# vlongle/pixie

Measured on NVIDIA H100. Metric: unet_voxels_per_s, higher is better.
Workload: dtype fp16e5 (U-Net, fp32 accumulate) + f32 (MPM)

## Files before the change

pixie_b200/csrc/conv3d_igemm.cu:

```cuda
#include "conv3d_igemm.cuh"
#include "ptx.cuh"

#include <algorithm>
#include <cmath>
#include <cstdio>
#include <cstring>

#include <cuda_fp8.h>

namespace pixie {

using namespace ptx;

namespace {

constexpr int kMaxWStages = 4;
constexpr int kMaxSStages = 8;
constexpr int kConsumerWarps = 8;
constexpr int kProducerWarp = 8;

struct SmemCtrl {
    uint64_t wfull[kMaxWStages];
    uint64_t wempty[kMaxWStages];
    uint64_t sfull[kMaxSStages];
    uint64_t sempty[kMaxSStages];
    int abort_flag;
};

constexpr int kCtlBarrierBytes = 512;
constexpr int kCmChunk = 16;
constexpr int kCmStageLd = 68;
constexpr int kCmStageFloats = kCmChunk * kCmStageLd;
constexpr int kStatsMaxC = 256;

struct TileCoord {
    int nb, d0, h0, w0, n0, ph_begin, ph_end, split, tde;
};

__device__ __forceinline__ TileCoord decode_tile(const ConvKernelParams& p, int wi) {
    TileCoord t;
    unsigned rest = (unsigned)wi;
    if (p.split_k == 1) {
        t.split = 0; t.ph_begin = 0; t.ph_end = p.n_phases;
    } else {
        const unsigned sk = (unsigned)p.split_k;
        t.split = (int)(rest % sk);
        rest /= sk;
        t.ph_begin = (int)(((unsigned)t.split * (unsigned)p.n_phases) / sk);
        t.ph_end = (int)((((unsigned)t.split + 1u) * (unsigned)p.n_phases) / sk);
    }
    const unsigned nt = rest % (unsigned)p.n_tiles;
    unsigned m = rest / (unsigned)p.n_tiles;
    const unsigned tw = m % (unsigned)p.tiles_w;
    m /= (unsigned)p.tiles_w;
    const unsigned th = m % (unsigned)p.tiles_h;
    m /= (unsigned)p.tiles_h;
    const unsigned td = m % (unsigned)p.tiles_d;
    t.nb = (int)(m / (unsigned)p.tiles_d);
    t.d0 = (int)td * p.TD;
    t.h0 = (int)th * p.TH;
    t.w0 = (int)tw * p.TW;
    t.n0 = (int)nt * p.block_n;
    t.tde = min(p.TD, p.D - t.d0);
    return t;
}

template <int N, bool F8>
__device__ __forceinline__ void mma_block(float* acc, uint32_t a, uint32_t b) {
    wgmma_fence();
#pragma unroll
    for (int k4 = 0; k4 < 4; ++k4) {
        const uint64_t da = make_sw128_desc(a + 32u * k4), db = make_sw128_desc(b + 32u * k4);
        if (F8) {
            if (N == 16) wgmma_e5m2_n16(acc, da, db);
            if (N == 32) wgmma_e5m2_n32(acc, da, db);
            if (N == 64) wgmma_e5m2_n64(acc, da, db);
            if (N == 128) wgmma_e5m2_n128(acc, da, db);
            if (N == 256) wgmma_e5m2_n256(acc, da, db);
        } else {
            if (N == 16) wgmma_f16_n16(acc, da, db);
            if (N == 32) wgmma_f16_n32(acc, da, db);
            if (N == 64) wgmma_f16_n64(acc, da, db);
            if (N == 128) wgmma_f16_n128(acc, da, db);
            if (N == 256) wgmma_f16_n256(acc, da, db);
        }
    }
    wgmma_commit();
}

__device__ __forceinline__ void wgmma_wait_n(int n) {
    switch (n) {
        case 0: wgmma_wait<0>(); break;
        case 1: wgmma_wait<1>(); break;
        case 2: wgmma_wait<2>(); break;
        case 3: wgmma_wait<3>(); break;
        case 4: wgmma_wait<4>(); break;
        case 5: wgmma_wait<5>(); break;
        case 6: wgmma_wait<6>(); break;
        case 7: wgmma_wait<7>(); break;
        case 8: wgmma_wait<8>(); break;
        case 9: wgmma_wait<9>(); break;
        default: wgmma_wait<0>(); break;
    }
}

struct RingPos {
    int stage = 0, parity = 0;
    __device__ __forceinline__ void advance(int n_stages) {
        if (++stage == n_stages) { stage = 0; parity ^= 1; }
    }
};

struct PendingStages {
    int s = -1, w = -1;
    __device__ __forceinline__ void release(SmemCtrl* ctl, int lane) {
        if (lane == 0) {
            if (s >= 0) mbar_arrive(&ctl->sempty[s]);
            if (w >= 0) mbar_arrive(&ctl->wempty[w]);
        }
        s = -1; w = -1;
    }
};

struct ConvStats {
    float* rows;
    int nb = -1;
    double tot_s = 0.0, tot_q = 0.0;

    __device__ __forceinline__ void flush(const ConvKernelParams& p, int lane) {
        if (p.stats_scalar) {
#pragma unroll
            for (int off = 16; off >= 1; off >>= 1) {
                tot_s += __shfl_xor_sync(0xffffffffu, tot_s, off);
                tot_q += __shfl_xor_sync(0xffffffffu, tot_q, off);
            }
            if (lane == 0) {
                atomicAdd(p.stats + (size_t)nb * p.Cout * 2, tot_s);
                atomicAdd(p.stats + (size_t)nb * p.Cout * 2 + 1, tot_q);
            }
            tot_s = 0.0; tot_q = 0.0;
            return;
        }
        asm volatile("bar.sync 1, 256;" ::: "memory");
        for (int ch = threadIdx.x; ch < p.Cout; ch += 256) {
            atomicAdd(p.stats + ((size_t)nb * p.Cout + ch) * 2, (double)rows[ch]);
            atomicAdd(p.stats + ((size_t)nb * p.Cout + ch) * 2 + 1, (double)rows[p.stats_ld + ch]);
            rows[ch] = 0.f;
            rows[p.stats_ld + ch] = 0.f;
        }
        asm volatile("bar.sync 1, 256;" ::: "memory");
    }
    __device__ __forceinline__ void enter(const ConvKernelParams& p, int item_nb, int lane) {
        if (nb != item_nb) {
            if (nb >= 0) flush(p, lane);
            nb = item_nb;
        }
    }
};

struct ConvSmem {
    uint8_t* w;
    uint8_t* s;
    SmemCtrl* ctl;
    float* stage;
    float* stats;
};

__device__ __forceinline__ ConvSmem conv_prologue(const ConvKernelParams& p, int stage_floats, int n_threads) {
    extern __shared__ __align__(1024) uint8_t smem_raw[];
    uint8_t* smem = reinterpret_cast<uint8_t*>(
        (reinterpret_cast<uintptr_t>(smem_raw) + 1023) & ~static_cast<uintptr_t>(1023));
    ConvSmem m;
    m.w = smem;
    m.s = smem + (size_t)p.w_stages * p.w_stage_bytes;
    m.ctl = reinterpret_cast<SmemCtrl*>(m.s + (size_t)p.s_stages * p.s_stage_bytes);
// ... 109 lines not shown
        RingPos wring, sring;
        const uint32_t w_base0 = smem_u32(sm.w), s_base0 = smem_u32(sm.s) + (uint32_t)(g * 64 * 128);
        bool ok = true;
        const long long DHW = (long long)p.D * p.H * p.W;
        ConvStats stats{sm.stats};
        int th2[2], tw2[2];
#pragma unroll
        for (int r2 = 0; r2 < 2; ++r2) {
            const int r = g * 64 + wq * 16 + (lane >> 2) + 8 * r2;
            th2[r2] = r / p.TW; tw2[r2] = r % p.TW;
        }
        const int cq = (lane & 3) * 2;

        for (int wi = blockIdx.x; wi < total_items && ok; wi += gridDim.x) {
            const TileCoord t = decode_tile(p, wi);
#pragma unroll
            for (int d = 0; d < TD; ++d)
#pragma unroll
                for (int j = 0; j < BN / 2; ++j) acc[d][j] = 0.f;
            PendingStages pend;
            int prev_f8 = -1;
            for (int ph = t.ph_begin; ph < t.ph_end && ok; ++ph) {
                const ConvPhase P = p.phases[ph];
                const int n_kd = P.n_kd, n_kh = P.n_kh;
                const bool f8 = P.f8 != 0;
                if (prev_f8 >= 0 && prev_f8 != (int)f8) wgmma_wait<0>();
                prev_f8 = (int)f8;
                ok = mbar_wait(&ctl->wfull[wring.stage], wring.parity, abort_flag);
                if (!ok) break;
                const uint32_t w_addr = w_base0 + (uint32_t)(wring.stage * p.w_stage_bytes);
                const int nplanes = t.tde + n_kd - 1;
                for (int pl = 0; pl < nplanes && ok; ++pl) {
                    ok = mbar_wait(&ctl->sfull[sring.stage], sring.parity, abort_flag);
                    if (!ok) break;
                    const int d_min = max(0, pl - (n_kd - 1)), d_max = min(t.tde - 1, pl);
                    const int groups = issue_slab<BN, TD>(acc, s_base0 + (uint32_t)(sring.stage * p.s_stage_bytes), w_addr, pl, d_min,
                                                          d_max, n_kd, n_kh, p.TW, f8);
                    wgmma_wait_n(groups);
                    pend.release(ctl, lane);
                    pend.s = sring.stage;
                    sring.advance(p.s_stages);
                }
                pend.w = wring.stage;
                wring.advance(p.w_stages);
                if (p.w_stages == 1) { wgmma_wait<0>(); pend.release(ctl, lane); }
            }
            wgmma_wait<0>();
            pend.release(ctl, lane);
#pragma unroll
            for (int d = 0; d < TD; ++d)
#pragma unroll
                for (int j = 0; j < BN / 2; ++j) fence_operand(acc[d][j]);
            if (!ok) break;

            if (do_stats) stats.enter(p, t.nb, lane);
            const bool first_split = (t.split == 0);
            const bool use_bias = first_split && p.bias != nullptr;
            const bool use_res = first_split && p.residual != nullptr;
#pragma unroll
            for (int d = 0; d < TD; ++d) {
                if (d >= t.tde) break;
#pragma unroll
                for (int r2 = 0; r2 < 2; ++r2) {
                    const int hh = t.h0 + th2[r2], ww = t.w0 + tw2[r2];
                    const bool row_ok = (hh < p.H) && (ww < p.W);
                    const long long vox = ((long long)(t.d0 + d) * p.H + hh) * p.W + ww;
#pragma unroll
                    for (int j8 = 0; j8 < BN / 8; ++j8) {
                        const int ch = t.n0 + j8 * 8 + cq;
                        float& a0 = acc[d][j8 * 4 + r2 * 2];
                        float& a1 = acc[d][j8 * 4 + r2 * 2 + 1];
                        const bool ok0 = row_ok && ch < p.Cout, ok1 = row_ok && ch + 1 < p.Cout;
                        float v0 = a0, v1 = a1;
                        if (use_bias) {
                            if (ok0) v0 += __ldg(p.bias + ch);
                            if (ok1) v1 += __ldg(p.bias + ch + 1);
                        }
                        if (p.out_planar) {
                            const long long i0 = ((long long)t.nb * p.Cout + ch) * DHW + vox;
                            if (ok0) {
                                if (use_res) v0 += p.residual[i0];
                                if (p.atomic_out) atomicAdd(p.out + i0, v0); else p.out[i0] = v0;
                            }
                            if (ok1) {
                                if (use_res) v1 += p.residual[i0 + DHW];
                                if (p.atomic_out) atomicAdd(p.out + i0 + DHW, v1); else p.out[i0 + DHW] = v1;
                            }
                        } else if (ok0) {
                            const long long base = ((long long)t.nb * DHW + vox) * p.out_ld + p.out_c0 + ch;
                            if (ok1 && (base & 1) == 0) {
                                if (use_res) {
                                    const float2 rv = __ldg(reinterpret_cast<const float2*>(p.residual + base));
                                    v0 += rv.x; v1 += rv.y;
                                }
                                if (p.atomic_out) red_add_v2(p.out + base, v0, v1);
                                else *reinterpret_cast<float2*>(p.out + base) = make_float2(v0, v1);
                            } else {
                                if (use_res) { v0 += p.residual[base]; if (ok1) v1 += p.residual[base + 1]; }
                                if (p.atomic_out) { atomicAdd(p.out + base, v0); if (ok1) atomicAdd(p.out + base + 1, v1); }
                                else { p.out[base] = v0; if (ok1) p.out[base + 1] = v1; }
                            }
                        }
                        a0 = ok0 ? v0 : 0.f;
                        a1 = ok1 ? v1 : 0.f;
                    }
                }
            }
            if (do_stats) {
                if (scalar_stats) {
                    float s = 0.f, q2 = 0.f;
#pragma unroll
                    for (int d = 0; d < TD; ++d)
#pragma unroll
                        for (int j = 0; j < BN / 2; ++j) { s += acc[d][j]; q2 = fmaf(acc[d][j], acc[d][j], q2); }
                    stats.tot_s += (double)s; stats.tot_q += (double)q2;
                } else {
#pragma unroll
                    for (int j8 = 0; j8 < BN / 8; ++j8)
#pragma unroll
                        for (int e = 0; e < 2; ++e) {
                            float s = 0.f, q2 = 0.f;
#pragma unroll
                            for (int d = 0; d < TD; ++d)
#pragma unroll
                                for (int r2 = 0; r2 < 2; ++r2) {
                                    const float v = acc[d][j8 * 4 + r2 * 2 + e];
                                    s += v; q2 = fmaf(v, v, q2);
                                }
#pragma unroll
                            for (int off = 4; off <= 16; off <<= 1) {
                                s += __shfl_xor_sync(0xffffffffu, s, off);
                                q2 += __shfl_xor_sync(0xffffffffu, q2, off);
                            }
                            const int ch = t.n0 + j8 * 8 + cq + e;
                            if (lane < 4 && ch < p.Cout) {
                                atomicAdd(stats.rows + ch, s);
                                atomicAdd(stats.rows + p.stats_ld + ch, q2);
                            }
                        }
                }
            }
        }
        if (do_stats && stats.nb >= 0 && ok) stats.flush(p, lane);
    }

    conv_report_abort(p, ctl);
}

template <int NV>
__global__ void __launch_bounds__(kConvCmThreads, 1)
conv3d_igemm_cm_kernel(const __grid_constant__ ConvKernelParams p) {
    constexpr int TW = NV == 64 ? 8 : 16;
    const ConvSmem sm = conv_prologue(p, 2 * kCmStageFloats, kConvCmThreads);
// ... 23 lines not shown
            const TileCoord t = decode_tile(p, wi);
#pragma unroll
            for (int j = 0; j < NV / 2; ++j) acc[j] = 0.f;
            const bool has_plane = g < t.tde;
            PendingStages pend;
            int prev_f8 = -1;
            for (int ph = t.ph_begin; ph < t.ph_end && ok; ++ph) {
                const ConvPhase P = p.phases[ph];
                const int n_kd = P.n_kd, n_kh = P.n_kh;
                const bool f8 = P.f8 != 0;
                if (prev_f8 >= 0 && prev_f8 != (int)f8) wgmma_wait<0>();
                prev_f8 = (int)f8;
                const int w0 = wring.stage;
                const int nplanes = t.tde + n_kd - 1;
                for (int pl = 0; pl < nplanes && ok; ++pl) {
                    if (pl < n_kd) {
                        ok = mbar_wait(&ctl->wfull[wring.stage], wring.parity, abort_flag);
                        if (!ok) break;
                        wring.advance(p.w_stages);
                    }
                    ok = mbar_wait(&ctl->sfull[sring.stage], sring.parity, abort_flag);
                    if (!ok) break;
                    const int kd = pl - g;
                    int groups = 0;
                    if (has_plane && kd >= 0 && kd < n_kd) {
                        int wsk = w0 + kd;
                        if (wsk >= p.w_stages) wsk -= p.w_stages;
                        const uint32_t w_addr = w_base0 + (uint32_t)(wsk * p.w_stage_bytes);
                        const uint32_t s_addr = s_base0 + (uint32_t)(sring.stage * p.s_stage_bytes);
                        for (int kh = 0; kh < n_kh; ++kh) {
                            const uint32_t a = w_addr + (uint32_t)(conv_wtile(0, 1, kh, 0) * 64 * 128);
                            const uint32_t b = s_addr + (uint32_t)(kh * TW * 128);
                            if (f8) mma_block<NV, true>(acc, a, b);
                            else mma_block<NV, false>(acc, a, b);
                            ++groups;
                        }
                    }
                    wgmma_wait_n(groups);
                    pend.release(ctl, lane);
                    pend.s = sring.stage;
                    const int kd_done = pl - t.tde + 1;
                    if (kd_done >= 0) {
                        pend.w = w0 + kd_done;
                        if (pend.w >= p.w_stages) pend.w -= p.w_stages;
                    }
                    sring.advance(p.s_stages);
                }
            }
            wgmma_wait<0>();
            pend.release(ctl, lane);
#pragma unroll
            for (int j = 0; j < NV / 2; ++j) fence_operand(acc[j]);
            if (!ok) break;

            if (do_stats) stats.enter(p, t.nb, lane);
            if (!has_plane) continue;
            const bool first_split = (t.split == 0);
            const int ch = t.n0 + 4 * q4;
            const bool ch_ok = ch < p.Cout;
            float4 bias4 = make_float4(0.f, 0.f, 0.f, 0.f);
            if (first_split && p.bias != nullptr && ch_ok)
                bias4 = make_float4(__ldg(p.bias + ch), __ldg(p.bias + ch + 1), __ldg(p.bias + ch + 2), __ldg(p.bias + ch + 3));
            const bool use_res = first_split && p.residual != nullptr;
            const long long plane_base = ((long long)t.nb * p.D + t.d0 + g) * p.H;
            float st_s[4] = {0.f, 0.f, 0.f, 0.f}, st_q[4] = {0.f, 0.f, 0.f, 0.f};
#pragma unroll
            for (int c = 0; c < NV / kCmChunk; ++c) {
#pragma unroll
                for (int jj = 0; jj < kCmChunk / 8; ++jj)
#pragma unroll
                    for (int r2 = 0; r2 < 2; ++r2)
#pragma unroll
                        for (int e = 0; e < 2; ++e) {
                            const int row = wq * 16 + (lane >> 2) + 8 * r2, v = jj * 8 + (lane & 3) * 2 + e;
                            stage[v * kCmStageLd + row] = acc[(c * (kCmChunk / 8) + jj) * 4 + r2 * 2 + e];
                        }
                asm volatile("bar.sync %0, 128;" ::"r"(2 + g) : "memory");
#pragma unroll
                for (int k = 0; k < kCmChunk / 8; ++k) {
                    const int v = vr + 8 * k, vt = c * kCmChunk + v;
                    const int hh = t.h0 + vt / TW, ww = t.w0 + vt % TW;
                    float4 x = *reinterpret_cast<const float4*>(stage + v * kCmStageLd + 4 * q4);
                    if (ch_ok && hh < p.H && ww < p.W) {
                        const long long base = ((plane_base + hh) * p.W + ww) * p.out_ld + p.out_c0 + ch;
                        x.x += bias4.x; x.y += bias4.y; x.z += bias4.z; x.w += bias4.w;
                        if (use_res) {
                            const float4 rv = __ldg(reinterpret_cast<const float4*>(p.residual + base));
                            x.x += rv.x; x.y += rv.y; x.z += rv.z; x.w += rv.w;
                        }
                        if (p.atomic_out) red_add_v4(p.out + base, x.x, x.y, x.z, x.w);
                        else *reinterpret_cast<float4*>(p.out + base) = x;
                        st_s[0] += x.x; st_s[1] += x.y; st_s[2] += x.z; st_s[3] += x.w;
                        st_q[0] = fmaf(x.x, x.x, st_q[0]); st_q[1] = fmaf(x.y, x.y, st_q[1]);
                        st_q[2] = fmaf(x.z, x.z, st_q[2]); st_q[3] = fmaf(x.w, x.w, st_q[3]);
                    }
                }
                asm volatile("bar.sync %0, 128;" ::"r"(2 + g) : "memory");
            }
            if (do_stats) {
                if (scalar_stats) {
                    stats.tot_s += (double)(st_s[0] + st_s[1] + st_s[2] + st_s[3]);
                    stats.tot_q += (double)(st_q[0] + st_q[1] + st_q[2] + st_q[3]);
                } else {
#pragma unroll
                    for (int i = 0; i < 4; ++i) {
                        st_s[i] += __shfl_xor_sync(0xffffffffu, st_s[i], 16);
                        st_q[i] += __shfl_xor_sync(0xffffffffu, st_q[i], 16);
                    }
                    if (lane < 16 && ch_ok) {
#pragma unroll
                        for (int i = 0; i < 4; ++i) {
                            atomicAdd(stats.rows + ch + i, st_s[i]);
                            atomicAdd(stats.rows + p.stats_ld + ch + i, st_q[i]);
                        }
                    }
                }
            }
        }
        if (do_stats && stats.nb >= 0 && ok) stats.flush(p, lane);
    }

    conv_report_abort(p, ctl);
}


int conv_k_total(const ConvDesc& d) {
    int k = 0;
    for (const auto& s : d.segs) k += s.ks * s.ks * s.ks * d.srcs[s.src].C;
    return k;
}

struct SrcSlot { int src; int n_kh; };

static std::vector<SrcSlot> conv_src_slots(const ConvDesc& d) {
    std::vector<SrcSlot> slots;
    for (const auto& s : d.segs) {
        const int n_kh = (s.ks == 3 && d.stride == 1) ? 3 : 1;
        bool found = false;
        for (const auto& sl : slots) found |= (sl.src == s.src && sl.n_kh == n_kh);
        if (!found) slots.push_back({s.src, n_kh});
    }
    return slots;
}

// ... 205 lines not shown

static bool vm_stages(const ConvKernelParams& p, int avail, int& ws, int& ss) {
    ws = (2 * p.w_stage_bytes + 2 * p.s_stage_bytes <= avail) ? 2 : 1;
    if (ws * p.w_stage_bytes + 2 * p.s_stage_bytes > avail) return false;
    ss = std::min(std::min(kMaxSStages, 6), (avail - ws * p.w_stage_bytes) / p.s_stage_bytes);
    return true;
}

int conv_plan_create(const ConvDesc& d, int* d_err_flag, ConvPlan& plan, char* err, int errlen) {
    auto fail = [&](const char* m) { snprintf(err, errlen, "conv_plan_create: %s", m); return 1; };
    PFN_encodeTiled enc = get_encode_fn();
    if (!enc) return fail("cuTensorMapEncodeTiled unavailable (no CUDA driver?)");
    if (d.srcs.empty() || d.segs.empty()) return fail("no sources/segments");
    for (const auto& s : d.srcs)
        if (s.C % 64) return fail("source channels must be a multiple of 64");
    if (d.Cout_pad % 16 || d.Cout_pad < d.Cout) return fail("Cout_pad must be a multiple of 16 >= Cout");

    ConvKernelParams& p = plan.p;
    memset(&p, 0, sizeof(p));
    p.NB = d.NB; p.D = d.D; p.H = d.H; p.W = d.W; p.stride = d.stride;
    p.Cout = d.Cout;
    const int out_ld = d.out_ld ? d.out_ld : d.Cout;

    const auto slots = conv_src_slots(d);
    if ((int)slots.size() > kConvMaxSrc) return fail("too many (source, tap-class) slots");
    const std::vector<ConvPhase> phases = conv_build_phases(d);
    p.n_phases = (int)phases.size();
    int max_taps = 1, max_kh = 1, max_kd = 1;
    bool any3 = false;
    for (const auto& P : phases) {
        max_taps = std::max(max_taps, P.n_kh * P.n_kd);
        max_kh = std::max(max_kh, (int)P.n_kh);
        max_kd = std::max(max_kd, (int)P.n_kd);
        any3 |= (P.n_kh == 3);
    }

    int dev = 0, sms = 132;
    cudaGetDevice(&dev);
    cudaDeviceGetAttribute(&sms, cudaDevAttrMultiProcessorCount, dev);

    plan.channel_major = d.Cout >= 64 && d.Cout % 4 == 0 && !d.out_planar && out_ld % 4 == 0 && d.out_c0 % 4 == 0 &&
                         reinterpret_cast<uintptr_t>(d.out) % 16 == 0 && reinterpret_cast<uintptr_t>(d.residual) % 16 == 0;
    const char* bad = plan.channel_major ? cm_geometry(d, sms, max_kh, p) : vm_geometry(d, sms, any3, max_taps, p);
    if (bad) return fail(bad);
    p.n_tiles = (d.Cout_pad + p.block_n - 1) / p.block_n;
    p.tiles_w = (d.W + p.TW - 1) / p.TW;
    p.tiles_h = (d.H + p.TH - 1) / p.TH;
    p.tiles_d = (d.D + p.TD - 1) / p.TD;

    const int items = conv_work_items(d.NB, p.tiles_d, p.tiles_h, p.tiles_w, p.n_tiles, 1);
    int split = d.split_k;
    if (split <= 0) {
        split = 1;
        while (items * split < 120 && split * 2 <= p.n_phases && split < 64) split *= 2;
    }
    split = std::max(1, std::min(split, p.n_phases));
    if ((long long)p.n_phases * (split + 1) >= (1ll << 31)) return fail("too many phases for the split-K bookkeeping");
    p.split_k = split;
    p.atomic_out = split > 1;
    plan.needs_zero = split > 1;

    for (size_t i = 0; i < slots.size(); ++i) p.slab_rows[i] = p.TW * (p.TH + slots[i].n_kh - 1);
    int max_rows = 0;
    for (size_t i = 0; i < slots.size(); ++i) max_rows = std::max(max_rows, p.slab_rows[i]);
    p.s_stage_bytes = max_rows * 128;
    plan.fused_stats = d.stats != nullptr && split == 1 && d.Cout <= kStatsMaxC && !d.out_planar;
    p.stats_ld = (d.Cout + 31) / 32 * 32;
    const int stats_bytes = plan.fused_stats ? 2 * p.stats_ld * 4 : 0;
    const int ctl_core = kCtlBarrierBytes + (plan.channel_major ? 2 * kCmStageFloats * 4 : 0) + stats_bytes;
    auto plan_stages = [&](int slack, int& ws, int& ss) {
        const int avail = 227 * 1024 - ctl_core - slack;
        return plan.channel_major ? cm_stages(p, max_kd, avail, ws, ss) : vm_stages(p, avail, ws, ss);
    };
    int ws1 = 0, ss1 = 0, ws0 = 0, ss0 = 0;
    const bool ok1 = plan_stages(1024, ws1, ss1), ok0 = plan_stages(0, ws0, ss0);
    if (!ok0) return fail("tile does not fit in shared memory");
    if (ok1 && ws1 >= ws0 && ss1 >= ss0) { p.smem_slack = 1024; p.w_stages = ws1; p.s_stages = ss1; }
    else { p.smem_slack = 0; p.w_stages = ws0; p.s_stages = ss0; }
    const int ctl_bytes = ctl_core + p.smem_slack;
    plan.smem_bytes = p.w_stages * p.w_stage_bytes + p.s_stages * p.s_stage_bytes + ctl_bytes;

    if (encode_a_maps(d, p, enc, err, errlen)) return 1;
    {
        const int K = conv_k_total(d);
        cuuint64_t gdim[2] = {(cuuint64_t)K, (cuuint64_t)d.Cout_pad};
        cuuint64_t gstr[1] = {(cuuint64_t)K * 2};
        cuuint32_t box[2] = {64, (cuuint32_t)p.block_n};
        cuuint32_t estr[2] = {1, 1};
        CUresult r = enc(&p.tmB, CU_TENSOR_MAP_DATA_TYPE_FLOAT16, 2, (void*)d.weights, gdim, gstr, box, estr,
                         CU_TENSOR_MAP_INTERLEAVE_NONE, CU_TENSOR_MAP_SWIZZLE_128B,
                         CU_TENSOR_MAP_L2_PROMOTION_L2_256B, CU_TENSOR_MAP_FLOAT_OOB_FILL_NONE);
        if (r != CUDA_SUCCESS) { snprintf(err, errlen, "cuTensorMapEncodeTiled(B) failed: %d", (int)r); return 1; }
    }

    if (cudaMalloc(&plan.d_phases, phases.size() * sizeof(ConvPhase)) != cudaSuccess) return fail("cudaMalloc phases");
    cudaMemcpy(plan.d_phases, phases.data(), phases.size() * sizeof(ConvPhase), cudaMemcpyHostToDevice);
    p.phases = plan.d_phases;

    p.bias = d.bias; p.residual = d.residual; p.out = d.out;
    p.out_ld = out_ld; p.out_c0 = d.out_c0; p.out_planar = d.out_planar;
    p.err_flag = d_err_flag;
    p.stats = plan.fused_stats ? d.stats : nullptr;
    p.stats_scalar = d.stats_scalar ? 1 : 0;
    plan.out_item_bytes = d.out_planar ? (size_t)d.Cout * d.D * d.H * d.W * 4
                                       : (size_t)d.D * d.H * d.W * p.out_ld * 4;

    plan.grid = std::min(items * split, sms);

    plan.kernel = plan.channel_major ? conv_cm_kernel_for(p.TH * p.TW) : conv_kernel_for(p.block_n, p.TD);
    plan.threads = plan.channel_major ? kConvCmThreads : kConvThreads;
    if (cudaFuncSetAttribute(plan.kernel, cudaFuncAttributeMaxDynamicSharedMemorySize, 227 * 1024) != cudaSuccess)
        return fail("cudaFuncSetAttribute(max dynamic smem)");
    return 0;
}

void conv_plan_destroy(ConvPlan& plan) {
    if (plan.d_phases) cudaFree(plan.d_phases);
    plan.d_phases = nullptr;
}

int conv_plan_launch(const ConvPlan& plan, int nb, cudaStream_t stream) {
    if (nb < 1 || nb > plan.p.NB) return (int)cudaErrorInvalidValue;
    ConvKernelParams p = plan.p;
    p.NB = nb;
    const int grid = std::min(plan.grid, conv_work_items(nb, p.tiles_d, p.tiles_h, p.tiles_w, p.n_tiles, p.split_k));
    if (plan.needs_zero) cudaMemsetAsync(p.out, 0, plan.out_item_bytes * (size_t)nb, stream);
    plan.kernel<<<grid, plan.threads, plan.smem_bytes, stream>>>(p);
    return (int)cudaGetLastError();
}

}
```

pixie_b200/csrc/conv3d_igemm.cuh:

```cuda
#pragma once
#include <cuda.h>
#include <cuda_runtime.h>
#include <cuda_fp16.h>
#include <cstdint>
#include <vector>

namespace pixie {

constexpr int kConvMaxSrc = 8;
constexpr int kF8Shift = 6;
constexpr int kConvThreads = 288;
constexpr int kConvCmThreads = 384;

struct ConvPhase {
    int8_t src;
    int8_t dw;
    int8_t dh0;
    int8_t dd0;
    int8_t n_kh;
    int8_t n_kd;
    int16_t c0;
    int32_t wtile_base;
    int32_t f8;
};
static_assert(sizeof(ConvPhase) == 16, "ConvPhase layout");

__host__ __device__ __forceinline__ int conv_wtile(int wtile_base, int n_kd, int kh, int kd) {
    return wtile_base + kh * n_kd + (n_kd - 1 - kd);
}

__host__ __device__ __forceinline__ int conv_work_items(int nb, int tiles_d, int tiles_h, int tiles_w, int n_tiles, int split_k) {
    return nb * tiles_d * tiles_h * tiles_w * n_tiles * split_k;
}

struct ConvKernelParams {
    CUtensorMap tmA[kConvMaxSrc];
    CUtensorMap tmB;
    const ConvPhase* phases;
    int n_phases;
    int split_k;
    int NB, D, H, W;
    int stride;
    int TW, TH, TD;
    int tiles_w, tiles_h, tiles_d;
    int Cout;
    int block_n;
    int n_tiles;
    int w_stage_bytes, w_stages;
    int s_stage_bytes, s_stages;
    int slab_rows[kConvMaxSrc];
    const float* bias;
    const float* residual;
    float* out;
    int out_ld;
    int out_c0;
    int out_planar;
    int atomic_out;
    double* stats;
    int stats_ld;
    int smem_slack;
    int stats_scalar;
    int* err_flag;
};

typedef void (*ConvKernelFn)(ConvKernelParams);

struct ConvSrc {
    const __half* ptr;
    int C;
    int Din, Hin, Win;
};

struct ConvDesc {
    int NB = 1;
    int D = 0, H = 0, W = 0;
    int stride = 1;
    int Cout = 0;
    struct Seg { int src; int ks; int wlo = 0; int f8 = 0; int lo = 0; };
    std::vector<ConvSrc> srcs;
    std::vector<Seg> segs;
    const __half* weights = nullptr;
    int Cout_pad = 0;
    const float* bias = nullptr;
    const float* residual = nullptr;
    float* out = nullptr;
    int out_ld = 0, out_c0 = 0, out_planar = 0;
    double* stats = nullptr;
    bool stats_scalar = false;
    int split_k = 1;
    int block_n = 0;
    int td = 0;
    int nv = 0;
};

int conv_k_total(const ConvDesc& d);

std::vector<ConvPhase> conv_build_phases(const ConvDesc& d);

void conv_pack_weights(const ConvDesc& d, const std::vector<const float*>& seg_weights,
                       const std::vector<int>& seg_cin_real, std::vector<__half>& packed);

struct ConvPlan {
    ConvKernelParams p{};
    ConvPhase* d_phases = nullptr;
    ConvKernelFn kernel = nullptr;
    bool channel_major = false;
    int threads = 0;
    int grid = 0;
    int smem_bytes = 0;
    bool needs_zero = false;
    bool fused_stats = false;
    size_t out_item_bytes = 0;
};

int conv_plan_create(const ConvDesc& d, int* d_err_flag, ConvPlan& plan, char* err, int errlen);
void conv_plan_destroy(ConvPlan& plan);
int conv_plan_launch(const ConvPlan& plan, int nb, cudaStream_t stream);
int conv_plan_retarget(const ConvDesc& d, ConvPlan& plan, char* err, int errlen);
}
```

pixie_b200/csrc/unet.cu:

```cuda
#include "unet.cuh"
#include "conv3d_igemm.cuh"
#include "unet_kernels.cuh"
#include "workspace.cuh"

#include <cmath>
#include <cstdio>
#include <cstdlib>
#include <cstring>
#include <functional>
#include <map>
#include <memory>
#include <string>
#include <vector>

namespace pixie {

namespace {

struct HostTensor {
    std::vector<float> data;
    std::vector<int64_t> shape;
};

struct ConvOp {
// ... 88 lines not shown
        }
        return &it->second;
    }
    size_t vox(int sp) const { return (size_t)sp * sp * sp; }

    double* stats_slot(int C) {
        double* s = u.d_stats + u.stats_doubles;
        u.stats_doubles += (size_t)NB * C * 2;
        return s;
    }

    struct F16 { __half* hi = nullptr; __half* lo = nullptr; int C = 0; int sp = 0; };

    F16 alloc_f16(int C, int sp) {
        F16 t; t.C = C; t.sp = sp;
        t.hi = dalloc<__half>((size_t)NB * vox(sp) * C);
        if (precise) t.lo = dalloc<__half>((size_t)NB * vox(sp) * C);
        return t;
    }

    void emit_moments(const DevT& x, double* stats) {
        UNet* up = &u;
        const int V = (int)vox(x.sp), C = x.C;
        const float* xp = x.p;
        u.ops.push_back([=](cudaStream_t st) { return launch_moments(xp, up->cur_nb, V, C, stats, st); });
        u.op_kinds.push_back(PIXIE_OP_MOMENTS); u.op_flops.push_back(0);
    }

    void emit_norm(const DevT& x, const double* stats, int mode, int groups, const float* gamma, const float* beta,
                   int act, const F16* dst, int c0, const F16* raw, int raw_c0) {
        NormArgs a;
        a.x = x.p; a.V = (int)vox(x.sp); a.C = x.C; a.stats = stats; a.mode = mode; a.groups = groups;

        a.gamma = gamma; a.beta = beta; a.eps = 1e-5f; a.act = act;
        a.lo_mode = f8corr ? 1 : 0;
        if (dst) { a.dst = dst->hi; a.dst_lo = dst->lo; a.dst_ld = dst->C; a.dst_c0 = c0; }
        if (raw) { a.raw_dst = raw->hi; a.raw_lo = raw->lo; a.raw_ld = raw->C; a.raw_c0 = raw_c0; }
        UNet* up = &u;
        u.ops.push_back([=](cudaStream_t st) { return launch_norm_act(a, up->cur_nb, st); });
        u.op_kinds.push_back(PIXIE_OP_NORM); u.op_flops.push_back(0);
    }

    struct ConvIn { F16 t; int ks; int cin_real; std::string wname; };

    ConvOp* emit_conv(const std::vector<ConvIn>& ins, int sp_out, int stride, int Cout, const float* residual,
                      float* out, bool planar, const std::vector<std::string>& bias_names, DevT* want_stats = nullptr) {
        if (!ok) return nullptr;
        auto op = std::make_unique<ConvOp>();
        const double flops_before = u.flops;
        ConvDesc& d = op->desc;
        d.NB = NB; d.D = d.H = d.W = sp_out; d.stride = stride; d.Cout = Cout;
        d.Cout_pad = (Cout + 15) / 16 * 16;
        d.split_k = 0;
        std::vector<const float*> wptr;
        std::vector<int> cin_real;
        std::vector<std::vector<float>> keep;
        for (const auto& in : ins) {
            const int ks = in.ks, kv = ks * ks * ks;
            const HostTensor* w = param(in.wname, (size_t)Cout * in.cin_real * kv);
            if (!w) return nullptr;
            const int si = (int)d.srcs.size();
            d.srcs.push_back({in.t.hi, in.t.C, in.t.sp, in.t.sp, in.t.sp});
            d.segs.push_back({si, ks, 0});
            wptr.push_back(w->data.data()); cin_real.push_back(in.cin_real);
            u.flops += 2.0 * (double)vox(sp_out) * Cout * in.cin_real * kv;
            if (f8corr && in.t.lo) {
                const int sl = (int)d.srcs.size();
                d.srcs.push_back({in.t.lo, in.t.C, in.t.sp, in.t.sp, in.t.sp});
                ConvDesc::Seg q{sl, ks, 0, 1};
                d.segs.push_back(q);
                wptr.push_back(w->data.data()); cin_real.push_back(in.cin_real);
            } else if (precise && in.t.lo) {
                const int sl = (int)d.srcs.size();
                d.srcs.push_back({in.t.lo, in.t.C, in.t.sp, in.t.sp, in.t.sp});
                d.segs.push_back({sl, ks, 0, 0, 1});
                wptr.push_back(w->data.data()); cin_real.push_back(in.cin_real);
                d.segs.push_back({si, ks, 1});
                wptr.push_back(w->data.data()); cin_real.push_back(in.cin_real);
            } else if (precise) {
                d.segs.push_back({si, ks, 1});
                wptr.push_back(w->data.data()); cin_real.push_back(in.cin_real);
            }
        }
        std::vector<__half> packed;
        conv_pack_weights(d, wptr, cin_real, packed);
        __half* dw = dalloc<__half>(packed.size());
        if (!dw) return nullptr;
        if (const cudaError_t e = cudaMemcpy(dw, packed.data(), packed.size() * 2, cudaMemcpyHostToDevice)) {
            fail("unet_finalize: cudaMemcpy", e);
            return nullptr;
        }
        d.weights = dw;
        std::vector<float> bias(Cout, 0.f);
        for (const auto& bn : bias_names) {
            const HostTensor* b = param(bn, (size_t)Cout);
            if (!b) return nullptr;
            for (int i = 0; i < Cout; ++i) bias[i] += b->data[i];
        }
        d.bias = upload(bias);
        d.residual = residual;
        d.out = out; d.out_ld = Cout; d.out_c0 = 0; d.out_planar = planar ? 1 : 0;
        if (want_stats) { want_stats->stats = stats_slot(Cout); d.stats = want_stats->stats; }
        char e[256] = {0};
        if (conv_plan_create(d, u.d_err, op->plan, e, sizeof(e))) {
            cudaGetLastError();
            fail(e);
// ... 161 lines not shown
        int ch = mc, sp = G, blk = 1;
        for (int level = 0; level < c.n_levels; ++level) {
            const int mult = c.channel_mult[level];
            for (int r = 0; r < c.num_res_blocks; ++r) {
                h = resblock({h}, mult * mc, "unet.input_blocks." + std::to_string(blk) + ".0");
                if (!h.p) return false;
                ch = mult * mc;
                hs.push_back(h);
                ++blk;
            }
            if (level != c.n_levels - 1) {
                h = downsample(h, "unet.input_blocks." + std::to_string(blk) + ".0");
                if (!h.p) return false;
                hs.push_back(h);
                ++blk;
                sp = (sp + 1) / 2;
            }
        }
        h = resblock({h}, ch, "unet.middle_block.0");
        if (!h.p) return false;
        h = attention(h, "unet.middle_block.1");
        if (!h.p) return false;
        h = resblock({h}, ch, "unet.middle_block.2");
        if (!h.p) return false;
        int ob = 0;
        for (int level = c.n_levels - 1; level >= 0; --level) {
            const int mult = c.channel_mult[level];
            for (int i = 0; i < c.num_res_blocks + 1; ++i) {
                DevT skip = hs.back();
                hs.pop_back();
                if (skip.sp != h.sp) return fail("odd grid sizes are not supported (crop path :925-930)");
                h = resblock({h, skip}, mc * mult, "unet.output_blocks." + std::to_string(ob) + ".0");
                if (!h.p) return false;
                if (level && i == c.num_res_blocks) {
                    h = upsample(h, "unet.output_blocks." + std::to_string(ob) + ".1");
                    if (!h.p) return false;
                }
                ++ob;
            }
        }
        {
            const size_t V = vox(G);
            const HostTensor *g = param("unet.out.0.weight", V), *b = param("unet.out.0.bias", V);
            if (!g || !b) return false;
            F16 a = alloc_f16(mc, G);
            if (!h.stats) return fail("internal: head input has no statistics");
            emit_norm(h, h.stats, kNormLN, 1, upload(g->data), upload(b->data), kActLeaky, &a, 0, nullptr, 0);
            u.out_staging = dalloc<float>((size_t)NB * c.out_channels * V);
            u.head_conv = emit_conv({{a, 3, mc, "unet.out.2.weight"}}, G, 1, c.out_channels, nullptr, u.out_staging, true, {"unet.out.2.bias"});
            if (!u.head_conv) return false;
        }
        if (u.stats_doubles > u.stats_cap) return fail("stats arena overflow");
        if (!ok) return false;
        const cudaError_t e = cudaDeviceSynchronize();
        return e == cudaSuccess || fail("unet_finalize", e);
    }
};

}

UNet* unet_create(const pixie_unet_config& cfg) {
    if (cfg.n_levels < 1 || cfg.n_levels > 8) { fail("n_levels out of range"); return nullptr; }
    if (cfg.grid_size % (1 << (cfg.n_levels - 1))) { fail("grid_size must be divisible by 2^(levels-1)"); return nullptr; }
    if (cfg.model_channels % 64) { fail("model_channels must be a multiple of 64"); return nullptr; }
    if (cfg.precision < 0 || cfg.precision > 2) { fail("precision must be 0 (fp16), 1 (fp16x3) or 2 (fp16 + e5m2 corrections)"); return nullptr; }
    auto* u = new UNet();
    u->cfg = cfg;
    u->use_graph = getenv("PIXIE_NO_GRAPH") == nullptr;
    u->NBmax = cfg.max_batch > 0 ? cfg.max_batch : 1;
    return u;
}

int unet_set_tensor(UNet* u, const char* name, const float* data, const int64_t* shape, int ndim) {
    if (u->finalized) return fail("set_tensor after finalize");
    HostTensor t;
    size_t n = 1;
    for (int i = 0; i < ndim; ++i) { t.shape.push_back(shape[i]); n *= (size_t)shape[i]; }
    t.data.assign(data, data + n);
    u->params[name] = std::move(t);
    return 0;
}

int unet_finalize(UNet* u) {
    if (u->finalized) return 0;
    Builder b(*u);
    if (!b.build()) return 1;
    u->params.clear();
    u->finalized = true;
    u->n_launch = (int)u->ops.size() + 1;
    return 0;
}

static int enqueue_ops(UNet* u, cudaStream_t st) {
    if (const cudaError_t e = cudaMemsetAsync(u->d_stats, 0, u->stats_doubles * sizeof(double), st)) return fail("unet_forward: statistics clear", e);
    for (auto& op : u->ops)
        if (const int rc = op(st)) return fail("unet_forward: kernel launch", (cudaError_t)rc);
    return 0;
}

static int run_ops(UNet* u, int batch, const void* feat, float* out, cudaStream_t st) {
    u->cur_nb = batch;
    if (u->use_graph) {
        UNet::GraphEntry* hit = nullptr;
        for (auto& g : u->graphs) if (g.exec && g.nb == batch && g.feat == feat && g.out == out) hit = &g;
        if (!hit) {
            UNet::GraphEntry& slot = u->graphs[u->graph_next];
// ... 68 lines not shown
    const cudaError_t e = time_ops(u, batch, st, ev, ms);
    for (cudaEvent_t x : ev) if (x) cudaEventDestroy(x);
    if (e != cudaSuccess) { fail("unet_profile", e); return -1; }
    for (int i = 0; i < n; ++i) {
        kinds[i] = u->op_kinds[i];
        flops[i] = u->op_flops[i];
    }
    return n;
}

int unet_forward_ncdhw(UNet* u, const float* feat_f32, int batch, float* out, cudaStream_t st) {
    if (!u->finalized) return fail("forward before finalize");
    if (batch < 1 || batch > u->NBmax) return fail("batch exceeds max_batch");
    const long long V = (long long)u->cfg.grid_size * u->cfg.grid_size * u->cfg.grid_size;
    if (const int rc = launch_ncdhw_to_ndhwc_f16(feat_f32, u->feat_staging, batch, u->cfg.feature_channels, u->feat_cpad, V, st))
        return fail("unet_forward_ncdhw: layout conversion", (cudaError_t)rc);
    return unet_forward(u, u->feat_staging, batch, out, st);
}

int unet_forward_host(UNet* u, const void* feat_host, int batch, float* out_host, cudaStream_t st) {
    if (!u->finalized) return fail("forward before finalize");
    if (batch < 1 || batch > u->NBmax) return fail("batch exceeds max_batch");
    if (u->feat_cpad != u->cfg.feature_channels) return fail("forward_host needs feature_channels % 64 == 0");
    const size_t V = (size_t)u->cfg.grid_size * u->cfg.grid_size * u->cfg.grid_size;
    if (const cudaError_t e = cudaMemcpyAsync(u->feat_staging, feat_host, (size_t)batch * V * u->feat_cpad * 2, cudaMemcpyHostToDevice, st))
        return fail("unet_forward_host: host-to-device copy", e);
    if (unet_forward(u, u->feat_staging, batch, u->out_staging, st)) return 1;
    if (const cudaError_t e = cudaMemcpyAsync(out_host, u->out_staging, (size_t)batch * u->cfg.out_channels * V * 4, cudaMemcpyDeviceToHost, st))
        return fail("unet_forward_host: device-to-host copy", e);
    if (const cudaError_t e = cudaStreamSynchronize(st)) return fail("unet_forward_host", e);
    return check_err_flag(u);
}

int64_t unet_debug_fetch(UNet* u, const char* name, float* host_out, int64_t capacity) {
    auto it = u->named.find(name);
    if (it == u->named.end()) { fail(std::string("no such activation: ") + name); return -1; }
    const DevT& t = it->second;
    const int64_t n = (int64_t)u->cur_nb * t.sp * t.sp * t.sp * t.C;
    if (n > capacity) { fail("debug_fetch: buffer too small"); return -2; }
    if (const cudaError_t e = cudaDeviceSynchronize()) { fail("unet_debug_fetch", e); return -3; }
    if (check_err_flag(u)) return -4;
    if (const cudaError_t e = cudaMemcpy(host_out, t.p, (size_t)n * 4, cudaMemcpyDeviceToHost)) { fail("unet_debug_fetch", e); return -3; }
    return n;
}

std::string unet_debug_names(UNet* u) {
    std::string s;
    for (const auto& kv : u->named)
        s += kv.first + " " + std::to_string(kv.second.C) + " " + std::to_string(kv.second.sp) + "\n";
    return s;
}

int unet_launch_count(UNet* u) {
    int n = 1;
    for (auto& c : u->convs) n += c->plan.needs_zero ? 1 : 0;
    return n + (int)u->ops.size();
}
double unet_flops(UNet* u) { return u->flops; }
int unet_check(UNet* u) {
    if (const cudaError_t e = cudaDeviceSynchronize()) return fail("unet_check", e);
    return check_err_flag(u);
}
void unet_destroy(UNet* u) { delete u; }

}
```

Measured before the change: 16.16 million.

## Replace atomic split-K output with workspace reduction by last-arriving CTA

Split-K partial accumulators are now written to a global workspace, and the last CTA to finish a tile (found through an atomic counter) sums all partials and runs the normal epilogue. This removes the output memset launch and the atomic adds to the output. It also lets fused statistics stay enabled when split-K is used. The split factor is now picked to fill the SMs well rather than by doubling to a fixed threshold. The cost is extra workspace traffic, a fence and barrier per tile, and a counter that has to be reset correctly across graph replays.

```diff
diff --git a/pixie_b200/csrc/conv3d_igemm.cu b/pixie_b200/csrc/conv3d_igemm.cu
--- a/pixie_b200/csrc/conv3d_igemm.cu
+++ b/pixie_b200/csrc/conv3d_igemm.cu
@@ -25,6 +25,7 @@
     uint64_t sfull[kMaxSStages];
     uint64_t sempty[kMaxSStages];
     int abort_flag;
+    int splitk_last;
 };
 
 constexpr int kCtlBarrierBytes = 512;
@@ -34,7 +35,7 @@
 constexpr int kStatsMaxC = 256;
 
 struct TileCoord {
-    int nb, d0, h0, w0, n0, ph_begin, ph_end, split, tde;
+    int tile, nb, d0, h0, w0, n0, ph_begin, ph_end, split, tde;
 };
 
 __device__ __forceinline__ TileCoord decode_tile(const ConvKernelParams& p, int wi) {
@@ -49,6 +50,7 @@
         t.ph_begin = (int)(((unsigned)t.split * (unsigned)p.n_phases) / sk);
         t.ph_end = (int)((((unsigned)t.split + 1u) * (unsigned)p.n_phases) / sk);
     }
+    t.tile = (int)rest;
     const unsigned nt = rest % (unsigned)p.n_tiles;
     unsigned m = rest / (unsigned)p.n_tiles;
     const unsigned tw = m % (unsigned)p.tiles_w;
@@ -121,6 +123,62 @@
         s = -1; w = -1;
     }
 };
+
+template <int N>
+__device__ __forceinline__ bool splitk_reduce(const ConvKernelParams& p, const TileCoord& t, float (&acc)[N], bool store,
+                                              SmemCtrl* ctl) {
+    static_assert(N % 4 == 0, "the accumulator is handed over as float4");
+    constexpr int kTileF4 = N / 4 * 256;
+    const int tid = threadIdx.x;
+    float4* ws = reinterpret_cast<float4*>(p.splitk_ws) + (size_t)t.tile * p.split_k * kTileF4 + tid;
+    if (store) {
+        float4* mine = ws + (size_t)t.split * kTileF4;
+#pragma unroll
+        for (int j = 0; j < N / 4; ++j)
+            __stcg(mine + j * 256, make_float4(acc[4 * j], acc[4 * j + 1], acc[4 * j + 2], acc[4 * j + 3]));
+    }
+    __threadfence();
+    asm volatile("bar.sync 1, 256;" ::: "memory");
+    if (tid == 0) {
+        const bool last = atomicAdd(p.splitk_count + t.tile, 1) == p.split_k - 1;
+        if (last) {
+            __threadfence();
+            p.splitk_count[t.tile] = 0;
+        }
+        ctl->splitk_last = last;
+    }
+    asm volatile("bar.sync 1, 256;" ::: "memory");
+    if (!ctl->splitk_last) return false;
+    if (!store) return true;
+#pragma unroll
+    for (int j = 0; j < N / 4; ++j) {
+        const float4 v = __ldcg(ws + j * 256);
+        acc[4 * j] = v.x; acc[4 * j + 1] = v.y; acc[4 * j + 2] = v.z; acc[4 * j + 3] = v.w;
+    }
+    int s = 1;
+    if constexpr (N <= 32) {
+        for (; s + 2 <= p.split_k; s += 2) {
+            float4 v0[N / 4], v1[N / 4];
+#pragma unroll
+            for (int j = 0; j < N / 4; ++j) {
+                v0[j] = __ldcg(ws + (size_t)s * kTileF4 + j * 256);
+                v1[j] = __ldcg(ws + (size_t)(s + 1) * kTileF4 + j * 256);
+            }
+#pragma unroll
+            for (int j = 0; j < N / 4; ++j) {
+                acc[4 * j] += v0[j].x; acc[4 * j + 1] += v0[j].y; acc[4 * j + 2] += v0[j].z; acc[4 * j + 3] += v0[j].w;
+                acc[4 * j] += v1[j].x; acc[4 * j + 1] += v1[j].y; acc[4 * j + 2] += v1[j].z; acc[4 * j + 3] += v1[j].w;
+            }
+        }
+    }
+    for (; s < p.split_k; ++s)
+#pragma unroll
+        for (int j = 0; j < N / 4; ++j) {
+            const float4 v = __ldcg(ws + (size_t)s * kTileF4 + j * 256);
+            acc[4 * j] += v.x; acc[4 * j + 1] += v.y; acc[4 * j + 2] += v.z; acc[4 * j + 3] += v.w;
+        }
+    return true;
+}
 
 struct ConvStats {
     float* rows;
@@ -336,11 +394,11 @@
 #pragma unroll
                 for (int j = 0; j < BN / 2; ++j) fence_operand(acc[d][j]);
             if (!ok) break;
+            if (p.split_k > 1 && !splitk_reduce(p, t, reinterpret_cast<float(&)[TD * (BN / 2)]>(acc), true, ctl)) continue;
 
             if (do_stats) stats.enter(p, t.nb, lane);
-            const bool first_split = (t.split == 0);
-            const bool use_bias = first_split && p.bias != nullptr;
-            const bool use_res = first_split && p.residual != nullptr;
+            const bool use_bias = p.bias != nullptr;
+            const bool use_res = p.residual != nullptr;
 #pragma unroll
             for (int d = 0; d < TD; ++d) {
                 if (d >= t.tde) break;
@@ -364,11 +422,11 @@
                             const long long i0 = ((long long)t.nb * p.Cout + ch) * DHW + vox;
                             if (ok0) {
                                 if (use_res) v0 += p.residual[i0];
-                                if (p.atomic_out) atomicAdd(p.out + i0, v0); else p.out[i0] = v0;
+                                p.out[i0] = v0;
                             }
                             if (ok1) {
                                 if (use_res) v1 += p.residual[i0 + DHW];
-                                if (p.atomic_out) atomicAdd(p.out + i0 + DHW, v1); else p.out[i0 + DHW] = v1;
+                                p.out[i0 + DHW] = v1;
                             }
                         } else if (ok0) {
                             const long long base = ((long long)t.nb * DHW + vox) * p.out_ld + p.out_c0 + ch;
@@ -377,12 +435,11 @@
                                     const float2 rv = __ldg(reinterpret_cast<const float2*>(p.residual + base));
                                     v0 += rv.x; v1 += rv.y;
                                 }
-                                if (p.atomic_out) red_add_v2(p.out + base, v0, v1);
-                                else *reinterpret_cast<float2*>(p.out + base) = make_float2(v0, v1);
+                                *reinterpret_cast<float2*>(p.out + base) = make_float2(v0, v1);
                             } else {
                                 if (use_res) { v0 += p.residual[base]; if (ok1) v1 += p.residual[base + 1]; }
-                                if (p.atomic_out) { atomicAdd(p.out + base, v0); if (ok1) atomicAdd(p.out + base + 1, v1); }
-                                else { p.out[base] = v0; if (ok1) p.out[base + 1] = v1; }
+                                p.out[base] = v0;
+                                if (ok1) p.out[base + 1] = v1;
                             }
                         }
                         a0 = ok0 ? v0 : 0.f;
@@ -512,16 +569,16 @@
 #pragma unroll
             for (int j = 0; j < NV / 2; ++j) fence_operand(acc[j]);
             if (!ok) break;
+            if (p.split_k > 1 && !splitk_reduce(p, t, acc, has_plane, ctl)) continue;
 
             if (do_stats) stats.enter(p, t.nb, lane);
             if (!has_plane) continue;
-            const bool first_split = (t.split == 0);
             const int ch = t.n0 + 4 * q4;
             const bool ch_ok = ch < p.Cout;
             float4 bias4 = make_float4(0.f, 0.f, 0.f, 0.f);
-            if (first_split && p.bias != nullptr && ch_ok)
+            if (p.bias != nullptr && ch_ok)
                 bias4 = make_float4(__ldg(p.bias + ch), __ldg(p.bias + ch + 1), __ldg(p.bias + ch + 2), __ldg(p.bias + ch + 3));
-            const bool use_res = first_split && p.residual != nullptr;
+            const bool use_res = p.residual != nullptr;
             const long long plane_base = ((long long)t.nb * p.D + t.d0 + g) * p.H;
             float st_s[4] = {0.f, 0.f, 0.f, 0.f}, st_q[4] = {0.f, 0.f, 0.f, 0.f};
 #pragma unroll
@@ -548,8 +605,7 @@
                             const float4 rv = __ldg(reinterpret_cast<const float4*>(p.residual + base));
                             x.x += rv.x; x.y += rv.y; x.z += rv.z; x.w += rv.w;
                         }
-                        if (p.atomic_out) red_add_v4(p.out + base, x.x, x.y, x.z, x.w);
-                        else *reinterpret_cast<float4*>(p.out + base) = x;
+                        *reinterpret_cast<float4*>(p.out + base) = x;
                         st_s[0] += x.x; st_s[1] += x.y; st_s[2] += x.z; st_s[3] += x.w;
                         st_q[0] = fmaf(x.x, x.x, st_q[0]); st_q[1] = fmaf(x.y, x.y, st_q[1]);
                         st_q[2] = fmaf(x.z, x.z, st_q[2]); st_q[3] = fmaf(x.w, x.w, st_q[3]);
@@ -861,19 +917,19 @@
     int split = d.split_k;
     if (split <= 0) {
         split = 1;
-        while (items * split < 120 && split * 2 <= p.n_phases && split < 64) split *= 2;
+        auto fill = [&](int s) { return (double)items * s / ((double)((items * s + sms - 1) / sms) * sms); };
+        if (items < 0.9 * sms)
+            while (fill(split) < 0.9 && split < p.n_phases) ++split;
     }
     split = std::max(1, std::min(split, p.n_phases));
     if ((long long)p.n_phases * (split + 1) >= (1ll << 31)) return fail("too many phases for the split-K bookkeeping");
     p.split_k = split;
-    p.atomic_out = split > 1;
-    plan.needs_zero = split > 1;
 
     for (size_t i = 0; i < slots.size(); ++i) p.slab_rows[i] = p.TW * (p.TH + slots[i].n_kh - 1);
     int max_rows = 0;
     for (size_t i = 0; i < slots.size(); ++i) max_rows = std::max(max_rows, p.slab_rows[i]);
     p.s_stage_bytes = max_rows * 128;
-    plan.fused_stats = d.stats != nullptr && split == 1 && d.Cout <= kStatsMaxC && !d.out_planar;
+    plan.fused_stats = d.stats != nullptr && d.Cout <= kStatsMaxC && !d.out_planar;
     p.stats_ld = (d.Cout + 31) / 32 * 32;
     const int stats_bytes = plan.fused_stats ? 2 * p.stats_ld * 4 : 0;
     const int ctl_core = kCtlBarrierBytes + (plan.channel_major ? 2 * kCmStageFloats * 4 : 0) + stats_bytes;
@@ -911,8 +967,18 @@
     p.err_flag = d_err_flag;
     p.stats = plan.fused_stats ? d.stats : nullptr;
     p.stats_scalar = d.stats_scalar ? 1 : 0;
-    plan.out_item_bytes = d.out_planar ? (size_t)d.Cout * d.D * d.H * d.W * 4
-                                       : (size_t)d.D * d.H * d.W * p.out_ld * 4;
+    if (split > 1) {
+        const size_t tile_floats = 256 * (size_t)(plan.channel_major ? p.TH * p.TW / 2 : p.TD * p.block_n / 2);
+        plan.splitk_ws_bytes = (size_t)items * split * tile_floats * 4;
+        plan.splitk_count_bytes = (size_t)items * sizeof(int);
+        if (!d.splitk_shared) {
+            if (cudaMalloc(&plan.splitk_buf, plan.splitk_ws_bytes + plan.splitk_count_bytes) != cudaSuccess)
+                return fail("cudaMalloc split-K workspace");
+            int* count = reinterpret_cast<int*>(reinterpret_cast<char*>(plan.splitk_buf) + plan.splitk_ws_bytes);
+            if (cudaMemset(count, 0, plan.splitk_count_bytes) != cudaSuccess) return fail("cudaMemset split-K counters");
+            conv_plan_bind_splitk(plan, reinterpret_cast<float*>(plan.splitk_buf), count);
+        }
+    }
 
     plan.grid = std::min(items * split, sms);
 
@@ -923,9 +989,16 @@
     return 0;
 }
 
+void conv_plan_bind_splitk(ConvPlan& plan, float* ws, int* count) {
+    plan.p.splitk_ws = ws;
+    plan.p.splitk_count = count;
+}
+
 void conv_plan_destroy(ConvPlan& plan) {
     if (plan.d_phases) cudaFree(plan.d_phases);
+    if (plan.splitk_buf) cudaFree(plan.splitk_buf);
     plan.d_phases = nullptr;
+    plan.splitk_buf = nullptr;
 }
 
 int conv_plan_launch(const ConvPlan& plan, int nb, cudaStream_t stream) {
@@ -933,7 +1006,6 @@
     ConvKernelParams p = plan.p;
     p.NB = nb;
     const int grid = std::min(plan.grid, conv_work_items(nb, p.tiles_d, p.tiles_h, p.tiles_w, p.n_tiles, p.split_k));
-    if (plan.needs_zero) cudaMemsetAsync(p.out, 0, plan.out_item_bytes * (size_t)nb, stream);
     plan.kernel<<<grid, plan.threads, plan.smem_bytes, stream>>>(p);
     return (int)cudaGetLastError();
 }
diff --git a/pixie_b200/csrc/conv3d_igemm.cuh b/pixie_b200/csrc/conv3d_igemm.cuh
--- a/pixie_b200/csrc/conv3d_igemm.cuh
+++ b/pixie_b200/csrc/conv3d_igemm.cuh
@@ -55,7 +55,8 @@
     int out_ld;
     int out_c0;
     int out_planar;
-    int atomic_out;
+    float* splitk_ws;
+    int* splitk_count;
     double* stats;
     int stats_ld;
     int smem_slack;
@@ -88,6 +89,7 @@
     double* stats = nullptr;
     bool stats_scalar = false;
     int split_k = 1;
+    bool splitk_shared = false;
     int block_n = 0;
     int td = 0;
     int nv = 0;
@@ -108,12 +110,13 @@
     int threads = 0;
     int grid = 0;
     int smem_bytes = 0;
-    bool needs_zero = false;
     bool fused_stats = false;
-    size_t out_item_bytes = 0;
+    size_t splitk_ws_bytes = 0, splitk_count_bytes = 0;
+    void* splitk_buf = nullptr;
 };
 
 int conv_plan_create(const ConvDesc& d, int* d_err_flag, ConvPlan& plan, char* err, int errlen);
+void conv_plan_bind_splitk(ConvPlan& plan, float* ws, int* count);
 void conv_plan_destroy(ConvPlan& plan);
 int conv_plan_launch(const ConvPlan& plan, int nb, cudaStream_t stream);
 int conv_plan_retarget(const ConvDesc& d, ConvPlan& plan, char* err, int errlen);
diff --git a/pixie_b200/csrc/unet.cu b/pixie_b200/csrc/unet.cu
--- a/pixie_b200/csrc/unet.cu
+++ b/pixie_b200/csrc/unet.cu
@@ -164,6 +164,7 @@
         d.NB = NB; d.D = d.H = d.W = sp_out; d.stride = stride; d.Cout = Cout;
         d.Cout_pad = (Cout + 15) / 16 * 16;
         d.split_k = 0;
+        d.splitk_shared = true;
         std::vector<const float*> wptr;
         std::vector<int> cin_real;
         std::vector<std::vector<float>> keep;
@@ -431,6 +432,20 @@
         }
         if (u.stats_doubles > u.stats_cap) return fail("stats arena overflow");
         if (!ok) return false;
+        {
+            size_t ws_bytes = 0, count_bytes = 0;
+            for (const auto& c : u.convs) {
+                ws_bytes = std::max(ws_bytes, c->plan.splitk_ws_bytes);
+                count_bytes = std::max(count_bytes, c->plan.splitk_count_bytes);
+            }
+            if (ws_bytes) {
+                float* ws = dalloc<float>(ws_bytes / 4);
+                int* count = dalloc<int>(count_bytes / sizeof(int));
+                if (!ws || !count) return false;
+                for (auto& c : u.convs)
+                    if (c->plan.splitk_ws_bytes) conv_plan_bind_splitk(c->plan, ws, count);
+            }
+        }
         const cudaError_t e = cudaDeviceSynchronize();
         return e == cudaSuccess || fail("unet_finalize", e);
     }
@@ -605,9 +620,7 @@
 }
 
 int unet_launch_count(UNet* u) {
-    int n = 1;
-    for (auto& c : u->convs) n += c->plan.needs_zero ? 1 : 0;
-    return n + (int)u->ops.size();
+    return 1 + (int)u->ops.size();
 }
 double unet_flops(UNet* u) { return u->flops; }
 int unet_check(UNet* u) {
```

New measurement: 16.17 million (median of 6 runs). Within noise of the previous version (+0.1%).
